# Visual-Behavior/aloception-oss

Hardware: AMD Instinct MI355X
Metric: frames/sec (whole node) DeformableDETR-R50 inference (higher is better)
Workload: dtype bf16; 1 GPU; DeformableDETR-R50 inference bf16, batch 8 synthetic 1333x800 frames per GPU, random-init weights; launch=hip-graph replay + eager inference(), per_gpu_batch=8, global_batch=8, parallelism=batch-sharded x1, no collective

## Files before the change

### aloception-oss_amd/alo_hip/__init__.py

```python
import ctypes
import warnings
import os
import subprocess

import torch

_PKG_ROOT = os.path.dirname(os.path.dirname(os.path.abspath(__file__)))
LIB_PATH = os.path.join(_PKG_ROOT, "libalo_hotpath.so")
CSRC_DIR = os.path.join(_PKG_ROOT, "csrc")

ALO_F32, ALO_F64, ALO_BF16, ALO_F16 = 0, 1, 2, 3
RESIDENT_AUTO, RESIDENT_ALWAYS = 0, 1
_DTYPE_CODE = {torch.float32: ALO_F32, torch.float64: ALO_F64, torch.bfloat16: ALO_BF16, torch.float16: ALO_F16}


def _half(f16):
    return (torch.bfloat16, torch.float16) if f16 else (torch.bfloat16,)


_lib = None
_warned_inference_tensor = False


def tensor_version(t):
# ... 747 lines not shown


def linear_packed(x, weight, bias=None, relu=False, residual=None):
    _no_autograd("linear_packed", x, weight, bias, residual)
    if not linear_packed_supported(x, weight, f16=True):
        raise RuntimeError("linear_packed: needs bf16 / fp16 CUDA tensors of one dtype, K % 256 == 0, K >= 512, N % 128 == 0, no autograd")
    x2 = x.reshape(-1, x.shape[-1])
    if not x2.is_contiguous():
        x2 = x2.contiguous()
    M, K = x2.shape
    N = weight.shape[0]
    y = torch.empty((M, N), dtype=x.dtype, device=x.device)
    if residual is not None:
        residual = residual.reshape(M, N)
        if residual.dtype != x.dtype or not residual.is_contiguous():
            raise RuntimeError("linear_packed: residual must be a contiguous (M, N) tensor of the input's dtype")
    if M:
        packed = pack_mfma_b(weight)
        bias_c = None if bias is None else bias.to(x.dtype).contiguous()
        _launch("alo_linear_packed", x.device, f"linear_packed/K={K}/N={N}", 2.0 * (M * K + M * N * (2 if residual is not None else 1)),
                2.0 * M * N * K, x2, packed, bias_c, residual, y, M, N, K, 1 if relu else 0, _DTYPE_CODE[x.dtype])
    return y.view(*x.shape[:-1], N)


def conv1x1_strided_supported(x, weight2d):
    if not (x.dim() == 4 and x.is_cuda and x.is_contiguous(memory_format=torch.channels_last)):
        return False
    if os.environ.get("ALO_CONV1X1_GATHER") == "0":
        return False
    rows = x.permute(0, 2, 3, 1)
    if linear_shortk_supported(rows, weight2d):
        return True
    return linear_packed_supported(rows, weight2d) and (weight2d.shape[0] >= 1024 or tuple(weight2d.shape) == (128, 512))


def conv1x1_strided(x, weight2d, bias, stride, relu=False):
    _no_autograd("conv1x1_strided", x, weight2d, bias)
    if not conv1x1_strided_supported(x, weight2d):
        raise RuntimeError("conv1x1_strided: unsupported dtype / layout / shape")
    n, cin, h, w_ = x.shape
    cout = weight2d.shape[0]
    ho, wo = (h - 1) // stride + 1, (w_ - 1) // stride + 1
    y = torch.empty((n, cout, ho, wo), dtype=x.dtype, device=x.device, memory_format=torch.channels_last)
    packed = not linear_shortk_supported(x.permute(0, 2, 3, 1), weight2d)
    wt = pack_mfma_b(weight2d) if packed else weight2d.contiguous()
    bias_c = None if bias is None else bias.to(x.dtype).contiguous()
    _launch("alo_conv1x1_nhwc", x.device, f"conv1x1_strided/K={cin}/N={cout}", 2.0 * (y.numel() // cout * cin + y.numel()),
            2.0 * y.numel() * cin, x, wt, 1 if packed else 0, bias_c, None, y, n, h, w_, cin, cout, stride, 1 if relu else 0, ALO_BF16)
    return y


CONV1X1_CHAIN, CONV1X1_CHAIN_DOWN = 2, 4


def bottleneck_chain_enabled():
    return os.environ.get("ALO_BOTTLENECK_CHAIN", "on").lower() not in ("off", "0")


def _chain_map(t, channels):
    return (t.dim() == 4 and t.is_cuda and t.dtype == torch.bfloat16 and t.shape[1] == channels and t.numel() > 0
            and t.is_contiguous(memory_format=torch.channels_last))


def _chain_vectors(*pairs):
    return all(w.dtype == torch.bfloat16 and tuple(w.shape[:2]) == (cout, cin) and w.numel() == cout * cin
               and b is not None and b.dtype == torch.bfloat16 and tuple(b.shape) == (cout,) for w, b, cout, cin in pairs)


def conv1x1_chain_supported(mid, conv3, identity=None, down=None, nxt=None):
    if (identity is None) == (down is None) or not bottleneck_chain_enabled() or torch.is_grad_enabled():
        return False
    other = identity if down is None else down[0]
    if not (_chain_map(mid, 64) and _chain_map(other, 256 if down is None else 64) and other.shape[0] == mid.shape[0]
            and other.shape[2:] == mid.shape[2:] and other.device == mid.device):
        return False
    pairs = [(*conv3, 256, 64)] + ([] if down is None else [(down[1], down[2], 256, 64)])
    if nxt is not None:
        if nxt[0].shape[0] not in (64, 128):
            return False
        pairs.append((*nxt, nxt[0].shape[0], 256))
    return _chain_vectors(*pairs) and fusable(mid, other, *[t for w, b, _, _ in pairs for t in (w, b)])


def conv1x1_chain(mid, conv3, identity=None, down=None, nxt=None):
    _no_autograd("conv1x1_chain", mid, *conv3, identity, *(down or ()), *(nxt or ()))
    if not conv1x1_chain_supported(mid, conv3, identity, down, nxt):
        raise RuntimeError("conv1x1_chain: needs channels-last bf16 CUDA maps outside autograd, a 64 -> 256 convolution, an identity or "
                           "a 64 -> 256 downsample convolution, a next convolution 256 -> 64 or 128, and ALO_BOTTLENECK_CHAIN not off")
    n, _, h, w_ = mid.shape
    n2 = 0 if nxt is None else nxt[0].shape[0]
    parts = [*conv3, *(down[1:] if down is not None else ()), *(nxt or ())]
    buf = derived(conv3[0], f"chain/{down is not None}/{n2}", parts, lambda: torch.cat([p.reshape(-1) for p in parts]))
    rows = n * h * w_
    out = torch.empty(rows * (256 + n2), dtype=mid.dtype, device=mid.device)
    other = identity if down is None else down[0]
    nbytes = 2.0 * rows * (64 + (256 if down is None else 64) + 256 + n2)
    flops = 2.0 * rows * 256 * (64 * (1 + (down is not None)) + n2)
    tag = f"conv1x1_chain/{'down' if down is not None else 'res'}{f'+next{n2}' if n2 else ''}"
    _launch("alo_conv1x1_nhwc", mid.device, tag, nbytes, flops, mid, buf, CONV1X1_CHAIN | (CONV1X1_CHAIN_DOWN if down is not None else 0) | n2,
            None, other, out, n, h, w_, 64, 256, 1, 1, ALO_BF16)
    y = out[:rows * 256].view(n, h, w_, 256).permute(0, 3, 1, 2)
    z = None if nxt is None else out[rows * 256:].view(n, h, w_, n2).permute(0, 3, 1, 2)
    return y, z


def f32_layers_split():
    return os.environ.get("ALO_F32_LAYERS") == "split"


_F32_ROUTED = {
    (64, 64): (0, None),
    (64, 256): (0, None),
    (256, 128): (0, 1 << 18),
    (256, 256): (0, 1 << 14),
    (256, 384): (0, None),
    (256, 512): (0, None),
    (256, 1024): (1 << 14, None),
    (512, 128): (0, None),
}


def _f32_gemm_routed(M, K, N, identity):
    if identity:
        return K <= 512
    lo, hi = _F32_ROUTED.get((K, N), (0, 0))
    return M >= lo and (hi is None or M < hi)


def linear_f32_supported(x, weight):
    return (x.is_cuda and x.dtype == torch.float32 and weight.dtype == torch.float32 and weight.dim() == 2 and x.dim() >= 1
            and x.shape[-1] == weight.shape[1] and weight.shape[1] % 64 == 0 and weight.shape[0] % 64 == 0 and weight.shape[0] > 0
            and weight.shape[1] > 0 and not needs_autograd(x, weight))


def linear_f32_routed(x, weight, identity=False):
    return (f32_layers_split() and linear_f32_supported(x, weight)
            and _f32_gemm_routed(x.numel() // max(x.shape[-1], 1), weight.shape[1], weight.shape[0], identity))


def _split_weight_of(weight):
    return derived(weight, "linear_f32_b", (weight,), lambda: _split_weight(weight))


def linear_f32(x, weight, bias=None, relu=False, residual=None):
    _no_autograd("linear_f32", x, weight, bias, residual)
    if not linear_f32_supported(x, weight):
        raise RuntimeError("linear_f32: needs fp32 CUDA tensors, a (N, K) weight, K % 64 == 0, N % 64 == 0, no autograd")
    N, K = weight.shape
    x2 = x.reshape(-1, K)
    if not x2.is_contiguous():
        x2 = x2.contiguous()
    M = x2.shape[0]
    y = torch.empty((M, N), dtype=x.dtype, device=x.device)
    if residual is not None:
        residual = residual.reshape(M, N)
# ... 904 lines not shown
```

### aloception-oss_amd/alonet/detr/backbone.py

```python
import torch
import torch.nn.functional as F
from torch import nn

import alo_hip

from .misc import assert_and_export_onnx


class FrozenBatchNorm2d(nn.Module):

    def __init__(self, n):
        super().__init__()
        self.register_buffer("weight", torch.ones(n))
        self.register_buffer("bias", torch.zeros(n))
        self.register_buffer("running_mean", torch.zeros(n))
        self.register_buffer("running_var", torch.ones(n))

    def _load_from_state_dict(self, state_dict, prefix, *args, **kwargs):
        state_dict.pop(prefix + "num_batches_tracked", None)
        super()._load_from_state_dict(state_dict, prefix, *args, **kwargs)

    def scale_shift(self):
        scale = self.weight * (self.running_var + 1e-5).rsqrt()
        return scale, self.bias - self.running_mean * scale
# ... 44 lines not shown
        w, b = folded_conv_bn(conv, bn)
        if alo_hip.fusable(x, w, b, residual) and x.is_contiguous(memory_format=torch.channels_last):
            if conv.kernel_size == (1, 1) and conv.padding == (0, 0) and conv.groups == 1 and w.shape[0] % 4 == 0:
                rows_probe = x.permute(0, 2, 3, 1)
                w2 = _weight_2d(w)
                if residual is None or (tuple(conv.stride) == (1, 1) and residual.is_contiguous(memory_format=torch.channels_last)
                                        and (alo_hip.linear_shortk_supported(rows_probe, w2)
                                             or alo_hip.linear_packed_supported(rows_probe, w2)
                                             or alo_hip.linear_f32_routed(rows_probe, w2, identity=True))):
                    return conv1x1_as_gemm(x, w, b, conv.stride, relu=relu, residual=residual)
                out = conv1x1_as_gemm(x, w, None, conv.stride)
                return alo_hip.bias_act_(out, b, residual, relu)
            dilated_ok = conv.dilation == (1, 1) or alo_hip.conv3x3_dilated_routed(x.dtype)
            if (residual is None and dilated_ok
                    and alo_hip.conv3x3_supported(x, w, conv.stride, conv.padding, conv.dilation, conv.groups)):
                return alo_hip.conv3x3(x, w, b, relu, conv.stride, **dilation_of(conv))
            if (residual is None and dilated_ok and alo_hip.f32_layers_split() and not (conv.stride == (2, 2) and w.shape[1] == 256)
                    and alo_hip.conv3x3_f32_supported(x, w, conv.stride, conv.padding, conv.dilation, conv.groups)):
                return alo_hip.conv3x3_f32(x, w, b, relu, conv.stride, **dilation_of(conv))
            if relu or residual is not None:
                out = F.conv2d(x, w, None, conv.stride, conv.padding, conv.dilation, conv.groups)
                if out.is_contiguous(memory_format=torch.channels_last) and out.shape[1] % 4 == 0:
                    return alo_hip.bias_act_(out, b, residual, relu)
                out = out + b.view(1, -1, 1, 1)
            else:
                out = F.conv2d(x, w, b, conv.stride, conv.padding, conv.dilation, conv.groups)
        else:
            out = F.conv2d(x, w, b, conv.stride, conv.padding, conv.dilation, conv.groups)
    else:
        out = bn(conv(x))
    if residual is not None:
        out = out + residual
    return F.relu_(out) if relu else out


_conv_bn = conv_bn


class Bottleneck(nn.Module):
    expansion = 4

    def __init__(self, inplanes, planes, stride=1, dilation=1, downsample=None, norm_layer=FrozenBatchNorm2d):
        super().__init__()
        self.conv1 = nn.Conv2d(inplanes, planes, 1, bias=False)
        self.bn1 = norm_layer(planes)
        self.conv2 = nn.Conv2d(planes, planes, 3, stride=stride, padding=dilation, dilation=dilation, bias=False)
        self.bn2 = norm_layer(planes)
        self.conv3 = nn.Conv2d(planes, planes * self.expansion, 1, bias=False)
        self.bn3 = norm_layer(planes * self.expansion)
        self.relu = nn.ReLU(inplace=True)
        self.downsample = downsample

    def _chain(self, x, mid, nxt):
        def pointwise(conv, bn):
            return (isinstance(bn, FrozenBatchNorm2d) and conv.bias is None and conv.kernel_size == (1, 1) and conv.stride == (1, 1)
                    and conv.padding == (0, 0) and conv.groups == 1)

        if not (conv_bn is _conv_bn and alo_hip.bottleneck_chain_enabled() and not torch.is_grad_enabled()
                and x.is_cuda and x.dtype == torch.bfloat16 and pointwise(self.conv3, self.bn3)
                and alo_hip.fusable(x, mid, self.conv3, self.bn3, self.downsample)):
            return None
        down = identity = head = None
        if self.downsample is None:
            identity = x
        elif len(self.downsample) == 2 and pointwise(self.downsample[0], self.downsample[1]):
            down = (x, *folded_conv_bn(self.downsample[0], self.downsample[1]))
        else:
            return None
        if isinstance(nxt, Bottleneck) and pointwise(nxt.conv1, nxt.bn1) and alo_hip.fusable(x, nxt.conv1, nxt.bn1):
            head = folded_conv_bn(nxt.conv1, nxt.bn1)
            if head[0].shape[0] not in (64, 128):
                head = None
        if down is None and head is None:
            return None
        args = (mid, folded_conv_bn(self.conv3, self.bn3), identity, down, head)
        return args if alo_hip.conv1x1_chain_supported(*args) else None

    def forward(self, x, head=None, nxt=None):
        out = conv_bn(x, self.conv1, self.bn1, relu=True) if head is None else head
        out = conv_bn(out, self.conv2, self.bn2, relu=True)
        chain = self._chain(x, out, nxt)
        if chain is not None:
            out, head = alo_hip.conv1x1_chain(*chain)
        else:
            identity = x if self.downsample is None else conv_bn(x, self.downsample[0], self.downsample[1])
            out, head = conv_bn(out, self.conv3, self.bn3, relu=True, residual=identity), None
        return out if nxt is None else (out, head)


_DEPTHS = {"resnet50": (3, 4, 6, 3), "resnet101": (3, 4, 23, 3)}


class ResNetBody(nn.Module):

    def __init__(self, name="resnet50", replace_stride_with_dilation=(False, False, False),
                 norm_layer=FrozenBatchNorm2d, return_layers=None):
        super().__init__()
        if name not in _DEPTHS:
            raise ValueError(f"backbone {name!r} is not available (have {sorted(_DEPTHS)})")
        self.inplanes, self.dilation = 64, 1
        self.conv1 = nn.Conv2d(3, 64, 7, stride=2, padding=3, bias=False)
        self.bn1 = norm_layer(64)
        self.relu = nn.ReLU(inplace=True)
        self.maxpool = nn.MaxPool2d(3, stride=2, padding=1)
        depths = _DEPTHS[name]
        self.layer1 = self._stage(64, depths[0], 1, False, norm_layer)
        self.layer2 = self._stage(128, depths[1], 2, replace_stride_with_dilation[0], norm_layer)
        self.layer3 = self._stage(256, depths[2], 2, replace_stride_with_dilation[1], norm_layer)
        self.layer4 = self._stage(512, depths[3], 2, replace_stride_with_dilation[2], norm_layer)
        self.return_layers = dict(return_layers or {"layer4": "0"})
        for m in self.modules():
            if isinstance(m, nn.Conv2d):
                nn.init.kaiming_normal_(m.weight, mode="fan_out", nonlinearity="relu")

    def _stage(self, planes, blocks, stride, dilate, norm_layer):
        prev_dilation = self.dilation
        if dilate:
            self.dilation *= stride
            stride = 1
        downsample = None
        if stride != 1 or self.inplanes != planes * Bottleneck.expansion:
            downsample = nn.Sequential(
                nn.Conv2d(self.inplanes, planes * Bottleneck.expansion, 1, stride=stride, bias=False),
                norm_layer(planes * Bottleneck.expansion))
        layers = [Bottleneck(self.inplanes, planes, stride, prev_dilation, downsample, norm_layer)]
        self.inplanes = planes * Bottleneck.expansion
# ... 89 lines not shown
```

### aloception-oss_amd/csrc/common.hpp

```cpp
#pragma once
#include <hip/hip_runtime.h>
#include <stdint.h>

#include <cstdarg>
#include <cstdio>
#include <type_traits>

#include "../../include/alo_hotpath.h"

namespace alo {

char* error_buffer();
inline int fail(alo_status_t code, const char* fmt, ...) {
    va_list ap;
    va_start(ap, fmt);
    vsnprintf(error_buffer(), 512, fmt, ap);
    va_end(ap);
    return (int)code;
}
#define ALO_REQUIRE(cond, code, ...) \
    do {                             \
        if (!(cond)) return ::alo::fail(code, __VA_ARGS__); \
    } while (0)

// ... 12 lines not shown
        static unsigned long long done = 0;
        int dev = 0;
        e = hipGetDevice(&dev);
        const unsigned long long bit = 1ull << (dev & 63);
        if (e == hipSuccess && !(__atomic_load_n(&done, __ATOMIC_ACQUIRE) & bit)) {
            e = hipFuncSetAttribute(fn, hipFuncAttributeMaxDynamicSharedMemorySize, kLdsLimit);
            if (e == hipSuccess) __atomic_fetch_or(&done, bit, __ATOMIC_RELEASE);
        }
    }
    if (e == hipSuccess) e = hipLaunchKernel(fn, grid, block, args, lds, stream);
    if (e == hipSuccess) e = hipGetLastError();
    if (e != hipSuccess) return fail(ALO_ERR_LAUNCH, "%s: %s", what, hipGetErrorString(e));
    return ALO_OK;
}

constexpr int kNumXcd = 8;

__device__ __forceinline__ unsigned xcd_contiguous_block(unsigned bid, unsigned nblocks) {
    const unsigned q = nblocks / kNumXcd, r = nblocks % kNumXcd;
    const unsigned xcd = bid % kNumXcd, k = bid / kNumXcd;
    const unsigned start = xcd < r ? xcd * (q + 1) : r * (q + 1) + (xcd - r) * q;
    return start + k;
}

static_assert(kNumXcd == 8, "the tile ranges below shift by 3");
struct TileRange { int first, end, step; };
__device__ __forceinline__ TileRange xcd_tile_range(int ntiles) {
    const int per_xcd = (ntiles + 7) >> 3, xcd = blockIdx.x & 7;
    const int end = (xcd + 1) * per_xcd < ntiles ? (xcd + 1) * per_xcd : ntiles;
    return {(int)(xcd * per_xcd + (blockIdx.x >> 3)), end, (int)(gridDim.x >> 3)};
}
inline unsigned xcd_grid(int ntiles, int max_per_xcd) {
    const int per_xcd = (ntiles + 7) / 8;
    return 8u * (unsigned)(per_xcd < max_per_xcd ? per_xcd : max_per_xcd);
}

struct WidePlan {
    int words[31];
};
bool msda_wide_plan(int N, int S, int M, int D, int Lq, int value_dtype, const int32_t* host_shapes, WidePlan* wp);
int msda_wide_launch(const void* value, const int32_t* shapes, const int32_t* lstart, const void* loc, const void* attn,
                     const void* grad_out, void* grad_value, void* grad_loc, void* grad_attn, const WidePlan& wp, int D,
                     int value_dtype, hipStream_t stream);

struct RowGather {
    int s, Wo, HoWo, W, HW;
};
inline RowGather row_gather(int stride = 1, int Ho = 1, int Wo = 1, int H = 1, int W = 1) { return {stride, Wo, Ho * Wo, W, H * W}; }

int linear_shortk_gather(const void* x, const void* weight, const void* bias, const void* residual, void* y, long M, int N, int K,
                         int relu, const RowGather& gather, hipStream_t stream);

int conv1x1_chain(const void* mid, const void* w_chain, const void* res_or_x0, void* y, long M, bool down, int n2, hipStream_t stream);

int conv3x3_f32(const void* x, const void* w_split, const void* bias, void* y, void* image_mag, int N, int H, int W, int Cin, int Cout,
                int stride, int dilation, int relu, hipStream_t stream);
int conv_taps_f32(const void* x, const void* w_split, const void* bias, void* y, void* image_mag, int N, int H, int W, int Cin, int Cout,
                  int vertical, int relu, hipStream_t stream);

int linear_f32(const void* x, const void* w_split, const void* bias, const void* residual, void* y, long M, int N, int K, int relu,
               const RowGather& gather, hipStream_t stream, const char* what);

int ffn_f32(const void* x, const void* w1_split, const void* b1, const void* w2_split, const void* b2, void* y, long M, int F,
            hipStream_t stream, const char* what);

int stem_conv_pool_f32(const void* x, const void* w_split, const void* bias, void* y, int N, int H, int W, long stride_n, long stride_c,
                       long stride_h, long stride_w, hipStream_t stream);

int instancenorm_f32(const void* x, void* y, void* workspace, int B, int HW, int C, float eps, long y_batch_stride, int relu,
                     hipStream_t stream, const char* what);

int upsample_flow_f32(const void* flow, const void* mask, void* out, int BQ, int C, int h, int w, hipStream_t stream, const char* what);
int upsample_flow_grad_f32(const void* flow_and_grad, const void* mask, void* out, int BQ, int C, int h, int w, hipStream_t stream,
                           const char* what);

int attention_block(const void* q, const void* k, const void* v, const void* mask, void* out, int batch, int S, int F, int pitch,
                    float scale, int dtype, hipStream_t stream, const char* what);

#define ALO_RELU_RES(fn, first, relu, residual, ...)                                                                          \
    ((residual) ? ((relu) ? fn<first, true, true>(__VA_ARGS__) : fn<first, false, true>(__VA_ARGS__))                          \
                : ((relu) ? fn<first, true, false>(__VA_ARGS__) : fn<first, false, false>(__VA_ARGS__)))

typedef __attribute__((ext_vector_type(4))) unsigned int u32x4;
typedef __attribute__((ext_vector_type(2))) unsigned int u32x2;
typedef __attribute__((ext_vector_type(4))) float f32x4;
typedef __attribute__((ext_vector_type(16))) float f32x16;

struct bf16_t {
    uint16_t bits;
};

__device__ __forceinline__ float relu_keep_nan(float v) { return (v > 0.f || v != v) ? v : 0.f; }

__device__ __forceinline__ float bf16_to_f32(uint16_t b) { return __uint_as_float(((unsigned)b) << 16); }
__device__ __forceinline__ uint16_t f32_to_bf16(float f) {
    const __bf16 b = static_cast<__bf16>(f);
    return __builtin_bit_cast(uint16_t, b);
}
__device__ __forceinline__ unsigned pack_bf16x2(float lo, float hi) {
    typedef __bf16 bf16x2_hw __attribute__((ext_vector_type(2)));
    typedef float f32x2_hw __attribute__((ext_vector_type(2)));
    const bf16x2_hw r = __builtin_convertvector(f32x2_hw{lo, hi}, bf16x2_hw);
    return __builtin_bit_cast(unsigned, r);
}

struct f16_t {
// ... 214 lines not shown
```

### aloception-oss_amd/csrc/gemm_packed.hip

```cpp
#include "mfma_tile.hpp"

namespace alo {
namespace {

constexpr int kOutStride = 64 * 2 + 16;

template <typename T, int kWC>
struct Packed {
    using type = T;
    static constexpr int WC = kWC;
};

struct PackedDims {
    long M;
    int N, K;
    RowGather g;
};

template <typename T, int WC, bool RELU, bool HAS_RES>
__global__ void __launch_bounds__(256, 2)
linear_packed_kernel(const T* __restrict__ X, const T* __restrict__ Wp, const T* __restrict__ bias, const T* __restrict__ R,
                     T* __restrict__ Y, const PackedDims dm) {
    constexpr int WR = 4 / WC;
    constexpr int kRows = 64 * WR;
// ... 83 lines not shown
    const dim3 grid((unsigned)((dm.M + kRows - 1) / kRows), (unsigned)(dm.N / (64 * WC)));
    return launch<linear_packed_kernel<typename Cfg::type, WC, RELU, HAS_RES>>(grid, 256, lds, stream, "alo_linear_packed", args);
}

template <typename T>
int dispatch_packed(const void* x, const void* w_packed, const void* bias, const void* residual, void* y, const PackedDims& dm,
                    int relu, void* stream) {
    hipStream_t s = static_cast<hipStream_t>(stream);
    using Wide = Packed<T, 4>;
    using Square = Packed<T, 2>;
    if (dm.N % 256 == 0) return ALO_RELU_RES(launch_packed, Wide, relu, residual, x, w_packed, bias, residual, y, dm, s);
    return ALO_RELU_RES(launch_packed, Square, relu, residual, x, w_packed, bias, residual, y, dm, s);
}

}
}

using namespace alo;

extern "C" int alo_linear_packed(const void* x, const void* w_packed, const void* bias, const void* residual, void* y, long M,
                                 int N, int K, int relu, int dtype, void* stream) {
    ALO_REQUIRE(dtype == ALO_BF16 || dtype == ALO_F16 || dtype == ALO_F32, ALO_ERR_UNSUPPORTED,
                "alo_linear_packed: bf16 / fp16, or fp32 with split weights, only (dtype %d)", dtype);
    ALO_REQUIRE(x && w_packed && y, ALO_ERR_INVALID_ARGUMENT, "alo_linear_packed: null pointer argument");
    ALO_REQUIRE(M > 0 && N > 0 && K > 0, ALO_ERR_INVALID_ARGUMENT, "alo_linear_packed: sizes must be positive");
    if (dtype == ALO_F32) {
        ALO_REQUIRE(K % 64 == 0 && N % 64 == 0, ALO_ERR_UNSUPPORTED, "alo_linear_packed: fp32 needs K and N to be multiples of 64 (K=%d N=%d)", K, N);
        ALO_REQUIRE(aligned16(x, w_packed, y, residual), ALO_ERR_INVALID_ARGUMENT, "alo_linear_packed: pointers must be 16-byte aligned");
        ALO_REQUIRE((M + 63) / 64 < (1L << 28), ALO_ERR_UNSUPPORTED, "alo_linear_packed: too many rows");
        return linear_f32(x, w_packed, bias, residual, y, M, N, K, relu, row_gather(), static_cast<hipStream_t>(stream), "alo_linear_packed");
    }
    ALO_REQUIRE(K % 256 == 0 && N % 128 == 0, ALO_ERR_UNSUPPORTED,
                "alo_linear_packed: K must be a multiple of 256 and N of 128 (K=%d N=%d)", K, N);
    ALO_REQUIRE(aligned16(x, w_packed, y, residual), ALO_ERR_INVALID_ARGUMENT, "alo_linear_packed: pointers must be 16-byte aligned");
    ALO_REQUIRE((M + 63) / 64 < (1L << 31), ALO_ERR_UNSUPPORTED, "alo_linear_packed: too many rows");
    PackedDims dm;
    dm.M = M; dm.N = N; dm.K = K; dm.g = row_gather();
    return with_storage_type(dtype, [&](auto t) { return dispatch_packed<decltype(t)>(x, w_packed, bias, residual, y, dm, relu, stream); });
}

extern "C" int alo_conv1x1_nhwc(const void* x, const void* weight, int weight_is_packed, const void* bias, const void* residual,
                                void* y, int N, int H, int W, int Cin, int Cout, int stride, int relu, int dtype, void* stream) {
    ALO_REQUIRE(x && weight && y, ALO_ERR_INVALID_ARGUMENT, "alo_conv1x1_nhwc: null pointer argument");
    ALO_REQUIRE(N > 0 && H > 0 && W > 0 && stride >= 1, ALO_ERR_INVALID_ARGUMENT, "alo_conv1x1_nhwc: N, H, W, stride must be positive");
    ALO_REQUIRE(dtype == ALO_BF16 || dtype == ALO_F32, ALO_ERR_UNSUPPORTED,
                "alo_conv1x1_nhwc: bf16 only, or fp32 with split packed weights (dtype %d)", dtype);
    ALO_REQUIRE(aligned16(x, weight, y, residual), ALO_ERR_INVALID_ARGUMENT, "alo_conv1x1_nhwc: pointers must be 16-byte aligned");
    const int Ho = (H - 1) / stride + 1, Wo = (W - 1) / stride + 1;
    const long M = (long)N * Ho * Wo;
    ALO_REQUIRE((long)H * W < (1L << 30), ALO_ERR_UNSUPPORTED, "alo_conv1x1_nhwc: map too large");
    if (weight_is_packed & ALO_CONV1X1_CHAIN) {
        const bool down = (weight_is_packed & ALO_CONV1X1_CHAIN_DOWN) != 0;
        const int n2 = weight_is_packed & ~(ALO_CONV1X1_CHAIN | ALO_CONV1X1_CHAIN_DOWN);
        ALO_REQUIRE(dtype == ALO_BF16 && Cin == 64 && Cout == 256 && stride == 1 && relu && (n2 == 0 || n2 == 64 || n2 == 128),
                    ALO_ERR_UNSUPPORTED,
                    "alo_conv1x1_nhwc: a chain buffer needs bf16, Cin = 64, Cout = 256, stride 1, relu and a next width of 0, 64 or 128 "
                    "(dtype %d Cin=%d Cout=%d stride=%d relu=%d next=%d)", dtype, Cin, Cout, stride, relu, n2);
        ALO_REQUIRE(residual && !bias, ALO_ERR_INVALID_ARGUMENT,
                    "alo_conv1x1_nhwc: a chain buffer carries its biases (bias must be NULL) and needs the identity, or the downsample "
                    "convolution's input, in residual");
        ALO_REQUIRE((M + 63) / 64 < (1L << 31), ALO_ERR_UNSUPPORTED, "alo_conv1x1_nhwc: too many output pixels");
        const size_t rows = (size_t)M;
        const struct { const void* p; size_t bytes; } out = {y, rows * 2 * (256 + (size_t)n2)},
                                                      ins[] = {{x, rows * 128}, {residual, rows * (down ? 128 : 512)}};
        for (const auto& i : ins)
            ALO_REQUIRE((const char*)out.p + out.bytes <= (const char*)i.p || (const char*)i.p + i.bytes <= (const char*)out.p,
                        ALO_ERR_INVALID_ARGUMENT, "alo_conv1x1_nhwc: the output of a chain overlaps an input");
        return conv1x1_chain(x, weight, residual, y, M, down, n2, static_cast<hipStream_t>(stream));
    }
    const RowGather gather = row_gather(stride, Ho, Wo, H, W);
    if (dtype == ALO_F32) {
        ALO_REQUIRE(weight_is_packed, ALO_ERR_UNSUPPORTED, "alo_conv1x1_nhwc: fp32 takes the split packed weight only (weight_is_packed = 1)");
        ALO_REQUIRE(Cin > 0 && Cout > 0 && Cin % 64 == 0 && Cout % 64 == 0, ALO_ERR_UNSUPPORTED,
                    "alo_conv1x1_nhwc: fp32 needs Cin and Cout to be multiples of 64 (Cin=%d Cout=%d)", Cin, Cout);
        ALO_REQUIRE((M + 63) / 64 < (1L << 28), ALO_ERR_UNSUPPORTED, "alo_conv1x1_nhwc: too many output pixels");
        return linear_f32(x, weight, bias, residual, y, M, Cout, Cin, relu, gather, static_cast<hipStream_t>(stream), "alo_conv1x1_nhwc");
    }
    if (!weight_is_packed) {
        ALO_REQUIRE(Cout % 64 == 0, ALO_ERR_UNSUPPORTED, "alo_conv1x1_nhwc: Cout must be a multiple of 64 (got %d)", Cout);
        return linear_shortk_gather(x, weight, bias, residual, y, M, Cout, Cin, relu, gather, static_cast<hipStream_t>(stream));
    }
    ALO_REQUIRE(Cin % 256 == 0 && Cout % 128 == 0, ALO_ERR_UNSUPPORTED,
                "alo_conv1x1_nhwc: packed weights need Cin %% 256 == 0 and Cout %% 128 == 0 (Cin=%d Cout=%d)", Cin, Cout);
    PackedDims dm;
    dm.M = M; dm.N = Cout; dm.K = Cin; dm.g = gather;
    return dispatch_packed<bf16_t>(x, weight, bias, residual, y, dm, relu, stream);
}
```

Measured before the change: 1001 frames/s.

## Extend fused bottleneck 1x1 chain kernel to ResNet layer2 (128->512)

Adds a new HIP kernel that fuses the layer2 bottleneck tail into one launch: the 128->512 conv3 with bias, the optional 256->512 downsample (stride 1 or 2 via a row gather) or residual add, ReLU, and the next block's 512->128 conv1. The aim is to avoid writing the 512-channel intermediate and reading it back across separate kernels, and to cut launch count in layer2. Python routing picks which layer2 variants use the chain, and the downsample and next-conv weights are packed into MFMA layout for it. It adds a large kernel with heavy LDS use and capped occupancy, which may run slower than the tuned separate GEMMs for some shapes.

```diff
diff --git a/aloception-oss_amd/alo_hip/__init__.py b/aloception-oss_amd/alo_hip/__init__.py
--- a/aloception-oss_amd/alo_hip/__init__.py
+++ b/aloception-oss_amd/alo_hip/__init__.py
@@ -823,9 +823,25 @@
 
 CONV1X1_CHAIN, CONV1X1_CHAIN_DOWN = 2, 4
 
+_CHAIN_FAMILIES = {64: (256, 64, (1,), (64, 128)), 128: (512, 256, (1, 2), (128,))}
+
+CHAIN_LAYER2_ROUTED = frozenset({(True, 128), (False, 128), (True, 0)})
+
+
+def _chain_knob():
+    return os.environ.get("ALO_BOTTLENECK_CHAIN", "on").lower()
+
 
 def bottleneck_chain_enabled():
-    return os.environ.get("ALO_BOTTLENECK_CHAIN", "on").lower() not in ("off", "0")
+    return _chain_knob() not in ("off", "0")
+
+
+def bottleneck_chain_routed(channels, down, n2):
+    if not bottleneck_chain_enabled():
+        return False
+    if channels == 64:
+        return True
+    return channels == 128 and _chain_knob() != "layer1" and (bool(down), int(n2)) in CHAIN_LAYER2_ROUTED
 
 
 def _chain_map(t, channels):
@@ -838,40 +854,63 @@
                and b is not None and b.dtype == torch.bfloat16 and tuple(b.shape) == (cout,) for w, b, cout, cin in pairs)
 
 
+def _chain_stride(down):
+    return 1 if down is None or len(down) < 4 else int(down[3])
+
+
 def conv1x1_chain_supported(mid, conv3, identity=None, down=None, nxt=None):
     if (identity is None) == (down is None) or not bottleneck_chain_enabled() or torch.is_grad_enabled():
         return False
+    if mid.dim() != 4 or mid.shape[1] not in _CHAIN_FAMILIES:
+        return False
+    cin = mid.shape[1]
+    cout, cin0, strides, widths = _CHAIN_FAMILIES[cin]
+    stride = _chain_stride(down)
+    if stride not in strides:
+        return False
     other = identity if down is None else down[0]
-    if not (_chain_map(mid, 64) and _chain_map(other, 256 if down is None else 64) and other.shape[0] == mid.shape[0]
-            and other.shape[2:] == mid.shape[2:] and other.device == mid.device):
+    if not (_chain_map(mid, cin) and _chain_map(other, cout if down is None else cin0) and other.shape[0] == mid.shape[0]
+            and tuple((d - 1) // stride + 1 for d in other.shape[2:]) == tuple(mid.shape[2:]) and other.device == mid.device):
         return False
-    pairs = [(*conv3, 256, 64)] + ([] if down is None else [(down[1], down[2], 256, 64)])
+    pairs = [(*conv3, cout, cin)] + ([] if down is None else [(down[1], down[2], cout, cin0)])
     if nxt is not None:
-        if nxt[0].shape[0] not in (64, 128):
+        if nxt[0].shape[0] not in widths:
             return False
-        pairs.append((*nxt, nxt[0].shape[0], 256))
+        pairs.append((*nxt, nxt[0].shape[0], cout))
     return _chain_vectors(*pairs) and fusable(mid, other, *[t for w, b, _, _ in pairs for t in (w, b)])
 
 
 def conv1x1_chain(mid, conv3, identity=None, down=None, nxt=None):
-    _no_autograd("conv1x1_chain", mid, *conv3, identity, *(down or ()), *(nxt or ()))
+    _no_autograd("conv1x1_chain", mid, *conv3, identity, *((down or ())[:3]), *(nxt or ()))
     if not conv1x1_chain_supported(mid, conv3, identity, down, nxt):
         raise RuntimeError("conv1x1_chain: needs channels-last bf16 CUDA maps outside autograd, a 64 -> 256 convolution, an identity or "
-                           "a 64 -> 256 downsample convolution, a next convolution 256 -> 64 or 128, and ALO_BOTTLENECK_CHAIN not off")
-    n, _, h, w_ = mid.shape
+                           "a 64 -> 256 downsample convolution, a next convolution 256 -> 64 or 128 (or 128 -> 512, a 256 -> 512 "
+                           "downsample convolution of stride 1 or 2, a next convolution 512 -> 128), and ALO_BOTTLENECK_CHAIN not off")
+    n, cin, h, w_ = mid.shape
+    cout, cin0 = _CHAIN_FAMILIES[cin][:2]
+    stride = _chain_stride(down)
     n2 = 0 if nxt is None else nxt[0].shape[0]
-    parts = [*conv3, *(down[1:] if down is not None else ()), *(nxt or ())]
-    buf = derived(conv3[0], f"chain/{down is not None}/{n2}", parts, lambda: torch.cat([p.reshape(-1) for p in parts]))
+    parts = [*conv3, *(down[1:3] if down is not None else ()), *(nxt or ())]
+
+    def chain_buffer():
+        flat = [p.reshape(-1) for p in parts]
+        if cin == 128:
+            for i in range(2, len(parts), 2):
+                flat[i] = _pack_mfma_b(parts[i].reshape(parts[i].shape[0], -1).contiguous()).reshape(-1)
+        return torch.cat(flat)
+
+    buf = derived(conv3[0], f"chain/{down is not None}/{n2}", parts, chain_buffer)
     rows = n * h * w_
-    out = torch.empty(rows * (256 + n2), dtype=mid.dtype, device=mid.device)
+    out = torch.empty(rows * (cout + n2), dtype=mid.dtype, device=mid.device)
     other = identity if down is None else down[0]
-    nbytes = 2.0 * rows * (64 + (256 if down is None else 64) + 256 + n2)
-    flops = 2.0 * rows * 256 * (64 * (1 + (down is not None)) + n2)
-    tag = f"conv1x1_chain/{'down' if down is not None else 'res'}{f'+next{n2}' if n2 else ''}"
+    nbytes = 2.0 * rows * (cin + (cout if down is None else cin0) + cout + n2)
+    flops = 2.0 * rows * cout * (cin + (cin0 if down is not None else 0) + n2)
+    form = f"{'down' if down is not None else 'res'}{f'+next{n2}' if n2 else ''}"
+    tag = f"conv1x1_chain/{form}" if cin == 64 else f"bottleneck_chain/C={cin}/{form}"
     _launch("alo_conv1x1_nhwc", mid.device, tag, nbytes, flops, mid, buf, CONV1X1_CHAIN | (CONV1X1_CHAIN_DOWN if down is not None else 0) | n2,
-            None, other, out, n, h, w_, 64, 256, 1, 1, ALO_BF16)
-    y = out[:rows * 256].view(n, h, w_, 256).permute(0, 3, 1, 2)
-    z = None if nxt is None else out[rows * 256:].view(n, h, w_, n2).permute(0, 3, 1, 2)
+            None, other, out, n, other.shape[2], other.shape[3], cin, cout, stride, 1, ALO_BF16)
+    y = out[:rows * cout].view(n, h, w_, cout).permute(0, 3, 1, 2)
+    z = None if nxt is None else out[rows * cout:].view(n, h, w_, n2).permute(0, 3, 1, 2)
     return y, z
 
 
diff --git a/aloception-oss_amd/alonet/detr/backbone.py b/aloception-oss_amd/alonet/detr/backbone.py
--- a/aloception-oss_amd/alonet/detr/backbone.py
+++ b/aloception-oss_amd/alonet/detr/backbone.py
@@ -120,26 +120,31 @@
         self.downsample = downsample
 
     def _chain(self, x, mid, nxt):
-        def pointwise(conv, bn):
-            return (isinstance(bn, FrozenBatchNorm2d) and conv.bias is None and conv.kernel_size == (1, 1) and conv.stride == (1, 1)
+        def pointwise(conv, bn, strides=((1, 1),)):
+            return (isinstance(bn, FrozenBatchNorm2d) and conv.bias is None and conv.kernel_size == (1, 1) and tuple(conv.stride) in strides
                     and conv.padding == (0, 0) and conv.groups == 1)
 
         if not (conv_bn is _conv_bn and alo_hip.bottleneck_chain_enabled() and not torch.is_grad_enabled()
                 and x.is_cuda and x.dtype == torch.bfloat16 and pointwise(self.conv3, self.bn3)
                 and alo_hip.fusable(x, mid, self.conv3, self.bn3, self.downsample)):
             return None
+        channels = self.conv3.in_channels
         down = identity = head = None
         if self.downsample is None:
             identity = x
-        elif len(self.downsample) == 2 and pointwise(self.downsample[0], self.downsample[1]):
-            down = (x, *folded_conv_bn(self.downsample[0], self.downsample[1]))
+        elif len(self.downsample) == 2 and pointwise(self.downsample[0], self.downsample[1], ((1, 1), (2, 2))):
+            down = (x, *folded_conv_bn(self.downsample[0], self.downsample[1]), self.downsample[0].stride[0])
         else:
             return None
         if isinstance(nxt, Bottleneck) and pointwise(nxt.conv1, nxt.bn1) and alo_hip.fusable(x, nxt.conv1, nxt.bn1):
             head = folded_conv_bn(nxt.conv1, nxt.bn1)
-            if head[0].shape[0] not in (64, 128):
+            if head[0].shape[0] not in ((64, 128) if channels == 64 else (128,)):
                 head = None
+        if head is not None and not alo_hip.bottleneck_chain_routed(channels, down is not None, head[0].shape[0]):
+            head = None
         if down is None and head is None:
+            return None
+        if not alo_hip.bottleneck_chain_routed(channels, down is not None, 0 if head is None else head[0].shape[0]):
             return None
         args = (mid, folded_conv_bn(self.conv3, self.bn3), identity, down, head)
         return args if alo_hip.conv1x1_chain_supported(*args) else None
diff --git a/aloception-oss_amd/csrc/common.hpp b/aloception-oss_amd/csrc/common.hpp
--- a/aloception-oss_amd/csrc/common.hpp
+++ b/aloception-oss_amd/csrc/common.hpp
@@ -88,6 +88,8 @@
                          int relu, const RowGather& gather, hipStream_t stream);
 
 int conv1x1_chain(const void* mid, const void* w_chain, const void* res_or_x0, void* y, long M, bool down, int n2, hipStream_t stream);
+int conv1x1_chain_l2(const void* mid, const void* w_chain, const void* res_or_x0, void* y, long M, bool down, int n2, const RowGather& gather,
+                     hipStream_t stream);
 
 int conv3x3_f32(const void* x, const void* w_split, const void* bias, void* y, void* image_mag, int N, int H, int W, int Cin, int Cout,
                 int stride, int dilation, int relu, hipStream_t stream);
diff --git a/aloception-oss_amd/csrc/conv1x1_chain_l2.hip b/aloception-oss_amd/csrc/conv1x1_chain_l2.hip
--- /dev/null
+++ b/aloception-oss_amd/csrc/conv1x1_chain_l2.hip
@@ -0,0 +1,319 @@
+#include "mfma_tile.hpp"
+
+namespace alo {
+namespace {
+
+constexpr int kRows = 64;
+constexpr int kK = 128;
+constexpr int kK0 = 256;
+constexpr int kN = 512;
+constexpr int kZN = 128;
+constexpr int kThreads = 512;
+constexpr int kInStride = kK * 2 + 16;
+constexpr int kIn0Stride = kK0 * 2 + 16;
+constexpr int kOutStride = 64 * 2 + 16;
+constexpr int kZStride = kZN * 2 + 16;
+constexpr int kSteps = kK / 16, kSteps0 = kK0 / 16, kNextSteps = kN / 16;
+constexpr int kPieces = kK / 8, kPieces0 = kK0 / 8, kZPieces = kZN / 8;
+constexpr int kLoads = kRows * kPieces / kThreads, kLoads0 = kRows * kPieces0 / kThreads;
+constexpr int kKB0 = 1;
+constexpr int kRing = 4;
+constexpr int kKB1 = 4;
+
+struct Chain2Args {
+    const bf16_t *X, *X0, *R;
+    const bf16_t *W3, *B3, *Wd, *Bd, *W1, *B1;
+    bf16_t *Y, *Z;
+    long M;
+    int tiles;
+    RowGather g;
+};
+
+constexpr size_t chain2_lds(bool down, bool next) {
+    return (size_t)kRows * kInStride + (down ? kRows * kIn0Stride : 0) + 8 * kRows * kOutStride + (next ? kRows * kZStride : 0) +
+           (8 * 64 * (down ? 2 : 1) + (next ? kZN : 0)) * sizeof(float);
+}
+
+template <int PIECES, int LOADS>
+__device__ __forceinline__ void park512(unsigned char* lds, int stride, const u32x4 (&v)[LOADS], int tid) {
+#pragma unroll
+    for (int j = 0; j < LOADS; ++j) {
+        const int p = tid + kThreads * j;
+        *reinterpret_cast<u32x4*>(lds + (p / PIECES) * stride + (p % PIECES) * 16) = v[j];
+    }
+}
+
+template <bool DOWN, bool NEXT>
+__global__ void __launch_bounds__(kThreads, 2) conv1x1_chain_l2_kernel(const Chain2Args a) {
+    using T = bf16_t;
+    static_assert(kRows * kPieces % kThreads == 0 && kRows * kPieces0 % kThreads == 0 && kRows * kZPieces % kThreads == 0,
+                  "the tile loaders give every thread the same number of pieces");
+    extern __shared__ __attribute__((aligned(16))) unsigned char smem[];
+    const int tid = threadIdx.x, wave = tid >> 6, lane = tid & 63;
+    const int nl = lane & 31, kg = lane >> 5;
+    unsigned char* const xbuf = smem;
+    unsigned char* const x0buf = smem + kRows * kInStride;
+    unsigned char* const ytile = x0buf + (DOWN ? kRows * kIn0Stride : 0);
+    unsigned char* const obuf = ytile + wave * (kRows * kOutStride);
+    unsigned char* const zbuf = ytile + 8 * kRows * kOutStride;
+    float* const tabs = reinterpret_cast<float*>(zbuf + (NEXT ? kRows * kZStride : 0));
+    float* const b3_tab = tabs + wave * 64;
+    float* const bd_tab = tabs + 8 * 64 + wave * 64;
+    float* const b1_tab = tabs + 8 * 64 * (DOWN ? 2 : 1);
+    const int col0 = wave * 64;
+
+    u32x4 w3[2][kSteps];
+#pragma unroll
+    for (int t = 0; t < 2; ++t)
+#pragma unroll
+        for (int s = 0; s < kSteps; ++s)
+            w3[t][s] = *reinterpret_cast<const u32x4*>(a.W3 + (size_t)(col0 + 32 * t + nl) * kK + 8 * kg + 16 * s);
+    {
+        const int r = lane & 15, t = (lane >> 4) & 1, k2 = lane >> 5;
+        const int c = col0 + 32 * t + (r & 3) + 8 * (r >> 2) + 4 * k2;
+        b3_tab[lane] = ld(&a.B3[c]);
+        if constexpr (DOWN) bd_tab[lane] = ld(&a.Bd[c]);
+    }
+    const int wave_u = __builtin_amdgcn_readfirstlane(wave);
+    unsigned lane_off = lane * 8;
+    [[maybe_unused]] const T* const wdp = DOWN ? a.Wd + (size_t)(2 * wave_u) * kSteps0 * 512 : nullptr;
+    auto load_wd = [&](u32x4 (&buf)[2][kKB0], int batch) {
+#pragma unroll
+        for (int t = 0; t < 2; ++t)
+#pragma unroll
+            for (int j = 0; j < kKB0; ++j) buf[t][j] = *reinterpret_cast<const u32x4*>(wdp + (t * kSteps0 + kKB0 * batch + j) * 512 + lane_off);
+        __builtin_amdgcn_sched_barrier(0);
+    };
+    const int zcol0 = 32 * (wave & 3), zhalf = wave >> 2;
+    [[maybe_unused]] const T* const w1p = NEXT ? a.W1 + (size_t)(wave_u & 3) * kNextSteps * 512 : nullptr;
+    auto load_w1 = [&](u32x4 (&buf)[kKB1], int batch) {
+#pragma unroll
+        for (int j = 0; j < kKB1; ++j) buf[j] = *reinterpret_cast<const u32x4*>(w1p + (kKB1 * batch + j) * 512 + lane_off);
+        __builtin_amdgcn_sched_barrier(0);
+    };
+    if constexpr (NEXT) {
+        if (tid < kZN) b1_tab[tid] = ld(&a.B1[tid]);
+    }
+
+    auto fetch = [&](int tile, u32x4 (&r)[kLoads]) {
+#pragma unroll
+        for (int j = 0; j < kLoads; ++j) {
+            const int p = tid + kThreads * j;
+            long row = (long)tile * kRows + p / kPieces;
+            row = row < a.M ? row : a.M - 1;
+            r[j] = *reinterpret_cast<const u32x4*>(a.X + row * kK + (p % kPieces) * 8);
+        }
+    };
+    auto fetch0 = [&](int tile, u32x4 (&r)[kLoads0]) {
+#pragma unroll
+        for (int j = 0; j < kLoads0; ++j) {
+            const int p = tid + kThreads * j;
+            long row = (long)tile * kRows + p / kPieces0;
+            row = gather_row(a.g, row < a.M ? row : a.M - 1);
+            r[j] = *reinterpret_cast<const u32x4*>(a.X0 + row * kK0 + (p % kPieces0) * 8);
+        }
+    };
+
+    int tile = blockIdx.x;
+    if (tile >= a.tiles) return;
+    u32x4 stage[kLoads];
+    [[maybe_unused]] u32x4 stage0[DOWN ? kLoads0 : 1];
+    [[maybe_unused]] u32x4 wd[kRing][2][kKB0];
+    fetch(tile, stage);
+    if constexpr (DOWN) {
+        fetch0(tile, stage0);
+#pragma unroll
+        for (int b = 0; b + 1 < kRing; ++b) load_wd(wd[b], b);
+    }
+
+    for (;;) {
+        asm volatile("" : "+v"(lane_off));
+        park512<kPieces>(xbuf, kInStride, stage, tid);
+        if constexpr (DOWN) park512<kPieces0>(x0buf, kIn0Stride, stage0, tid);
+        __syncthreads();
+        const long grow0 = (long)tile * kRows;
+        const int next = tile + gridDim.x;
+        const bool more = next < a.tiles;
+        [[maybe_unused]] u32x4 idn[DOWN ? 1 : 8];
+        if constexpr (!DOWN) fetch_identity(idn, a.R, grow0, a.M, kN, col0, lane);
+        if (more) {
+            fetch(next, stage);
+        }
+
+        [[maybe_unused]] unsigned dpk[DOWN ? 2 : 1][2][8];
+        if constexpr (DOWN) {
+            f32x16 accd[2][2];
+#pragma unroll
+            for (int t = 0; t < 2; ++t)
+#pragma unroll
+                for (int q = 0; q < 4; ++q) {
+                    const f32x4 d4 = *reinterpret_cast<const f32x4*>(bd_tab + (kg * 2 + t) * 16 + 4 * q);
+#pragma unroll
+                    for (int i = 0; i < 4; ++i) accd[0][t][4 * q + i] = accd[1][t][4 * q + i] = d4[i];
+                }
+            auto mma_wd = [&](const u32x4 (&buf)[2][kKB0], int batch) {
+                u32x4 af[2][kKB0];
+#pragma unroll
+                for (int j = 0; j < kKB0; ++j) {
+                    const int s = kKB0 * batch + j;
+                    af[0][j] = *reinterpret_cast<const u32x4*>(x0buf + nl * kIn0Stride + (16 * s + 8 * kg) * 2);
+                    af[1][j] = *reinterpret_cast<const u32x4*>(x0buf + (32 + nl) * kIn0Stride + (16 * s + 8 * kg) * 2);
+                }
+#pragma unroll
+                for (int j = 0; j < kKB0; ++j)
+#pragma unroll
+                    for (int h = 0; h < 2; ++h)
+#pragma unroll
+                        for (int t = 0; t < 2; ++t) accd[h][t] = mfma_32x32x16<T>(buf[t][j], af[h][j], accd[h][t]);
+                __builtin_amdgcn_sched_barrier(0);
+            };
+#pragma unroll
+            for (int bt = 0; bt < kSteps0; ++bt) {
+                load_wd(wd[(bt + kRing - 1) % kRing], (bt + kRing - 1) % kSteps0);
+                mma_wd(wd[bt % kRing], bt);
+            }
+#pragma unroll
+            for (int h = 0; h < 2; ++h)
+#pragma unroll
+                for (int t = 0; t < 2; ++t)
+#pragma unroll
+                    for (int i = 0; i < 8; ++i) dpk[h][t][i] = pack2<T>(accd[h][t][2 * i], accd[h][t][2 * i + 1]);
+            if (more) fetch0(next, stage0);
+        }
+
+#pragma unroll
+        for (int half = 0; half < kRows / 32; ++half) {
+            f32x16 acc[2];
+#pragma unroll
+            for (int t = 0; t < 2; ++t)
+#pragma unroll
+                for (int q = 0; q < 4; ++q) {
+                    const f32x4 b4 = *reinterpret_cast<const f32x4*>(b3_tab + (kg * 2 + t) * 16 + 4 * q);
+#pragma unroll
+                    for (int i = 0; i < 4; ++i) acc[t][4 * q + i] = b4[i];
+                }
+#pragma unroll
+            for (int s = 0; s < kSteps; ++s) {
+                const u32x4 f = *reinterpret_cast<const u32x4*>(xbuf + (32 * half + nl) * kInStride + (16 * s + 8 * kg) * 2);
+                acc[0] = mfma_32x32x16<T>(w3[0][s], f, acc[0]);
+                acc[1] = mfma_32x32x16<T>(w3[1][s], f, acc[1]);
+            }
+            if constexpr (DOWN) {
+#pragma unroll
+                for (int t = 0; t < 2; ++t)
+#pragma unroll
+                    for (int q = 0; q < 4; ++q) {
+                        unsigned o[2];
+#pragma unroll
+                        for (int i = 0; i < 2; ++i) {
+                            float plo, phi, dlo, dhi;
+                            unpack2<T>(pack2<T>(acc[t][4 * q + 2 * i], acc[t][4 * q + 2 * i + 1]), plo, phi);
+                            unpack2<T>(dpk[half][t][2 * q + i], dlo, dhi);
+                            o[i] = pack2<T>(relu_keep_nan(plo + dlo), relu_keep_nan(phi + dhi));
+                        }
+                        *reinterpret_cast<u32x2*>(obuf + (32 * half + nl) * kOutStride + (32 * t + 8 * q + 4 * kg) * 2) = u32x2{o[0], o[1]};
+                    }
+            } else {
+                stage_quads<T, false>(obuf, kOutStride, acc, nullptr, false, 32 * half + nl, 0, kg);
+            }
+        }
+        [[maybe_unused]] u32x4 w1a[kKB1], w1b[kKB1];
+        if constexpr (NEXT) load_w1(w1a, 0);
+        wave_lds_fence();
+#pragma unroll
+        for (int pass = 0; pass < 8; ++pass) {
+            const int row = pass * 8 + (lane >> 3);
+            unsigned char* const at = obuf + row * kOutStride + (lane & 7) * 16;
+            u32x4 v = *reinterpret_cast<const u32x4*>(at);
+            if constexpr (!DOWN) {
+                v = add_residual_x8<T, true>(v, idn[pass]);
+                if constexpr (NEXT) *reinterpret_cast<u32x4*>(at) = v;
+            }
+            if (grow0 + row < a.M) *reinterpret_cast<u32x4*>(a.Y + (grow0 + row) * kN + col0 + (lane & 7) * 8) = v;
+        }
+
+        if constexpr (NEXT) {
+            __syncthreads();
+            f32x16 accz;
+#pragma unroll
+            for (int i = 0; i < 16; ++i) accz[i] = 0.f;
+            const unsigned char* const yrow = ytile + (32 * zhalf + nl) * kOutStride + 8 * kg * 2;
+            auto mma_w1 = [&](const u32x4 (&buf)[kKB1], int batch) {
+                u32x4 af[kKB1];
+#pragma unroll
+                for (int j = 0; j < kKB1; ++j) {
+                    const int s = kKB1 * batch + j;
+                    af[j] = *reinterpret_cast<const u32x4*>(yrow + (s >> 2) * (kRows * kOutStride) + 16 * (s & 3) * 2);
+                }
+#pragma unroll
+                for (int j = 0; j < kKB1; ++j) accz = mfma_32x32x16<T>(buf[j], af[j], accz);
+                __builtin_amdgcn_sched_barrier(0);
+            };
+            constexpr int kBatches = kNextSteps / kKB1;
+#pragma unroll
+            for (int bt = 0; bt < kBatches; bt += 2) {
+                load_w1(w1b, bt + 1);
+                mma_w1(w1a, bt);
+                if (bt + 2 < kBatches) load_w1(w1a, bt + 2);
+                mma_w1(w1b, bt + 1);
+            }
+#pragma unroll
+            for (int q = 0; q < 4; ++q) {
+                const int c = zcol0 + 8 * q + 4 * kg;
+                const f32x4 bb = *reinterpret_cast<const f32x4*>(b1_tab + c);
+                float v0 = accz[4 * q], v1 = accz[4 * q + 1], v2 = accz[4 * q + 2], v3 = accz[4 * q + 3];
+                v0 += bb[0]; v1 += bb[1]; v2 += bb[2]; v3 += bb[3];
+                v0 = relu_keep_nan(v0); v1 = relu_keep_nan(v1); v2 = relu_keep_nan(v2); v3 = relu_keep_nan(v3);
+                *reinterpret_cast<u32x2*>(zbuf + (32 * zhalf + nl) * kZStride + c * 2) = u32x2{pack2<T>(v0, v1), pack2<T>(v2, v3)};
+            }
+            __syncthreads();
+#pragma unroll
+            for (int j = 0; j < kRows * kZPieces / kThreads; ++j) {
+                const int p = tid + kThreads * j, row = p / kZPieces, piece = p % kZPieces;
+                if (grow0 + row < a.M)
+                    *reinterpret_cast<u32x4*>(a.Z + (grow0 + row) * kZN + piece * 8) =
+                        *reinterpret_cast<const u32x4*>(zbuf + row * kZStride + piece * 16);
+            }
+            if (!more) break;
+        } else {
+            if (!more) break;
+            __syncthreads();
+        }
+        tile = next;
+    }
+}
+
+template <bool DOWN, bool NEXT>
+int launch_chain2(const Chain2Args& a, hipStream_t stream) {
+    int gx = a.tiles < 256 ? a.tiles : 256;
+    void* args[] = {const_cast<Chain2Args*>(&a)};
+    return launch<conv1x1_chain_l2_kernel<DOWN, NEXT>>(gx, kThreads, chain2_lds(DOWN, NEXT), stream, "alo_conv1x1_nhwc", args);
+}
+
+}
+}
+
+int alo::conv1x1_chain_l2(const void* mid, const void* w_chain, const void* res_or_x0, void* y, long M, bool down, int n2,
+                          const RowGather& gather, hipStream_t stream) {
+    const bf16_t* w = static_cast<const bf16_t*>(w_chain);
+    Chain2Args a{};
+    a.X = static_cast<const bf16_t*>(mid);
+    (down ? a.X0 : a.R) = static_cast<const bf16_t*>(res_or_x0);
+    a.W3 = w; w += kN * kK;
+    a.B3 = w; w += kN;
+    if (down) {
+        a.Wd = w; w += kN * kK0;
+        a.Bd = w; w += kN;
+    }
+    if (n2) {
+        a.W1 = w; w += (size_t)kZN * kN;
+        a.B1 = w;
+    }
+    a.Y = static_cast<bf16_t*>(y);
+    a.Z = n2 ? a.Y + M * kN : nullptr;
+    a.M = M;
+    a.tiles = (int)((M + kRows - 1) / kRows);
+    a.g = gather;
+    if (down) return n2 ? launch_chain2<true, true>(a, stream) : launch_chain2<true, false>(a, stream);
+    return n2 ? launch_chain2<false, true>(a, stream) : launch_chain2<false, false>(a, stream);
+}
diff --git a/aloception-oss_amd/csrc/gemm_packed.hip b/aloception-oss_amd/csrc/gemm_packed.hip
--- a/aloception-oss_amd/csrc/gemm_packed.hip
+++ b/aloception-oss_amd/csrc/gemm_packed.hip
@@ -159,21 +159,25 @@
     if (weight_is_packed & ALO_CONV1X1_CHAIN) {
         const bool down = (weight_is_packed & ALO_CONV1X1_CHAIN_DOWN) != 0;
         const int n2 = weight_is_packed & ~(ALO_CONV1X1_CHAIN | ALO_CONV1X1_CHAIN_DOWN);
-        ALO_REQUIRE(dtype == ALO_BF16 && Cin == 64 && Cout == 256 && stride == 1 && relu && (n2 == 0 || n2 == 64 || n2 == 128),
-                    ALO_ERR_UNSUPPORTED,
-                    "alo_conv1x1_nhwc: a chain buffer needs bf16, Cin = 64, Cout = 256, stride 1, relu and a next width of 0, 64 or 128 "
+        const bool l1 = Cin == 64 && Cout == 256 && stride == 1 && (n2 == 0 || n2 == 64 || n2 == 128);
+        const bool l2 = Cin == 128 && Cout == 512 && (stride == 1 || (stride == 2 && down)) && (n2 == 0 || n2 == 128);
+        ALO_REQUIRE(dtype == ALO_BF16 && relu && (l1 || l2), ALO_ERR_UNSUPPORTED,
+                    "alo_conv1x1_nhwc: a chain buffer needs bf16, Cin = 64, Cout = 256, stride 1, relu and a next width of 0, 64 or 128, "
+                    "or Cin = 128, Cout = 512, stride 1 (2 with _DOWN) and a next width of 0 or 128 "
                     "(dtype %d Cin=%d Cout=%d stride=%d relu=%d next=%d)", dtype, Cin, Cout, stride, relu, n2);
         ALO_REQUIRE(residual && !bias, ALO_ERR_INVALID_ARGUMENT,
                     "alo_conv1x1_nhwc: a chain buffer carries its biases (bias must be NULL) and needs the identity, or the downsample "
                     "convolution's input, in residual");
         ALO_REQUIRE((M + 63) / 64 < (1L << 31), ALO_ERR_UNSUPPORTED, "alo_conv1x1_nhwc: too many output pixels");
         const size_t rows = (size_t)M;
-        const struct { const void* p; size_t bytes; } out = {y, rows * 2 * (256 + (size_t)n2)},
-                                                      ins[] = {{x, rows * 128}, {residual, rows * (down ? 128 : 512)}};
+        const size_t other = !down ? rows * 2 * (size_t)Cout : l1 ? rows * 128 : (size_t)N * H * W * 512;
+        const struct { const void* p; size_t bytes; } out = {y, rows * 2 * ((size_t)Cout + (size_t)n2)},
+                                                      ins[] = {{x, rows * 2 * (size_t)Cin}, {residual, other}};
         for (const auto& i : ins)
             ALO_REQUIRE((const char*)out.p + out.bytes <= (const char*)i.p || (const char*)i.p + i.bytes <= (const char*)out.p,
                         ALO_ERR_INVALID_ARGUMENT, "alo_conv1x1_nhwc: the output of a chain overlaps an input");
-        return conv1x1_chain(x, weight, residual, y, M, down, n2, static_cast<hipStream_t>(stream));
+        if (l1) return conv1x1_chain(x, weight, residual, y, M, down, n2, static_cast<hipStream_t>(stream));
+        return conv1x1_chain_l2(x, weight, residual, y, M, down, n2, row_gather(stride, Ho, Wo, H, W), static_cast<hipStream_t>(stream));
     }
     const RowGather gather = row_gather(stride, Ho, Wo, H, W);
     if (dtype == ALO_F32) {
```

After: 1020 frames/s, median of 6. +1.9%, better.
